# 17LiQi/MultimodalSignal

Hardware: AMD Instinct MI355X
Metric: train windows/sec (higher is better)
Workload: dtype f32; 1 GPU; CnnGruAttentionModel full train step (fwd+CE+bwd+Adam, dropout 0.5, BN batch stats), B=8192 windows/GPU x (6 ch, 3840 samples = 60 s @ 64 Hz), random-init weights; BASELINE.json configs[4] shape, the per-step work of configs[1]; batch_per_gpu=8192, channels=6, samples=3840, classes=2, parallelism=replica x1

## Files before the change

### multimodalsignal_amd/csrc/gru_bwd4.h

```cpp
#pragma once
template <int I> struct BwdB4 {
  static constexpr bool L1K = (I == 128);
  static constexpr int SD = 288;
  static constexpr int SX = L1K ? 224 : 96;
  static constexpr int DGP = 16 * SD, XHP = 16 * SX;
  static constexpr int BUFE = 3 * DGP + 3 * XHP;
  static constexpr int NPC = 6, NST = L1K ? 2 : 3;
  static constexpr int STG0 = 2 * BUFE * 2;
  static constexpr int SLOTB = 4 * NPC * 1024;
  static constexpr int SMEM = STG0 + NST * SLOTB;
};
struct BwdB6 {
  static constexpr int SD = 288, SX = 96, DGP = 16 * SD, XHP = 16 * SX;
  static constexpr int DGBUF = 3 * DGP, XHBUF = 3 * XHP;
  static constexpr int XH0 = 2 * DGBUF, NXH = 4;
  static constexpr int HNH0 = (XH0 + NXH * XHBUF) * 2;
  static constexpr int STG0 = HNH0 + 2 * 4096;
  static constexpr int NPC = 4, NST = 2, SLOTB = 4 * NPC * 1024;
  static constexpr int WHN0 = STG0 + NST * SLOTB;
  static constexpr int SMEM = WHN0 + 2 * 12288;
};
struct GruArgs;
struct FoldCtx;
int launch_gru_bwd_b4(int I, bool folds, const GruArgs& a, int n_tiles, int nwg, int ndir, const FoldCtx& fc, hipStream_t st, bool waves8 = false);
int launch_gru_bwd_seq4(int dh_mode, const GruArgs& a, int n_tiles, int ndir, const FoldCtx& fc, hipStream_t st);
int launch_gru_bwd_seq4_dw1(const GruArgs& a, const GruArgs& a1, int n_tiles, int nwg1, const FoldCtx& fc, hipStream_t st);
int gru_bwd_b4_lds_optin();
int launch_gru_bwd_b6(bool folds, const GruArgs& a, int n_tiles, int nwg, int ndir, const FoldCtx& fc, hipStream_t st);
int gru_bwd_b6_lds_optin();
```

### multimodalsignal_amd/csrc/gru_bwd6.hip

```cpp
#include "gru_args.h"
#include "gru_bwd4.h"
#include "gru_bwd_pipe.h"

template <bool FOLDS, int ROLE>
__device__ __forceinline__ void bwd6_run(const GruArgs& a, const GruDir& D, const float* __restrict__ ax_, const uint32_t dkey, const int n_tiles) {
  using G = BwdB6;
  constexpr int I = 32;
  constexpr bool CH = ROLE == 0, BA = ROLE == 1, BB = ROLE == 2;
  constexpr int SD = G::SD, SX = G::SX, DGP = G::DGP, XHP = G::XHP, DGBUF = G::DGBUF, XHBUF = G::XHBUF, XH0 = G::XH0;
  extern __shared__ __attribute__((aligned(16))) __bf16 ring[];
  constexpr int NT = BA ? 3 : (BB ? 6 : 0), NTA = NT > 0 ? NT : 1;
  constexpr int NST = G::NST, SLOTB = G::SLOTB, NPIECE = 4;
  const int tid = threadIdx.x, lane = tid & 63, w = (tid >> 6) & 3, li = lane & 15, lq = lane >> 4;
  const int u0 = w * 16 + lq * 4;

  bf16x8 AhB[CH ? 6 : 1][3], AiB[BA ? 6 : 1][3];
  if constexpr (CH || BA) {
#pragma unroll
    for (int kb = 0; kb < 6; ++kb)
#pragma unroll
      for (int j = 0; j < 8; ++j) {
        __bf16 p0, p1, p2;
        if constexpr (CH) {
          split3(D.Whh[(size_t)(kb * 32 + lq * 8 + j) * 64 + w * 16 + li], p0, p1, p2);
          AhB[kb][0][j] = p0; AhB[kb][1][j] = p1; AhB[kb][2][j] = p2;
        } else {
          split3(D.Wih[(size_t)(kb * 32 + lq * 8 + j) * I + w * 16 + li], p0, p1, p2);
          AiB[kb][0][j] = p0; AiB[kb][1][j] = p1; AiB[kb][2][j] = p2;
        }
      }
#pragma unroll
    for (int kb = 0; kb < 6; ++kb)
#pragma unroll
      for (int pp = 0; pp < 3; ++pp) { if constexpr (CH) PIN_ACC(AhB[kb][pp]); else PIN_ACC(AiB[kb][pp]); }
  }
  f32x4 b_hn[2] = {{0.f, 0.f, 0.f, 0.f}, {0.f, 0.f, 0.f, 0.f}};
  char* const whn = (char*)ring + G::WHN0 + (w & 1) * 12288 + lane * 16;
  if constexpr (BA) {
#pragma unroll
    for (int ub = 0; ub < 2; ++ub) {
#pragma unroll
      for (int kb = 0; kb < 2; ++kb) {
        const float* wr = D.Whh + (size_t)(128 + (w + 2 * ub) * 16 + li) * 64 + kb * 32 + lq * 8;
        bf16x8 P[3];
#pragma unroll
        for (int j = 0; j < 8; ++j) { __bf16 p0, p1, p2; split3(wr[j], p0, p1, p2); P[0][j] = p0; P[1][j] = p1; P[2][j] = p2; }
#pragma unroll
        for (int pp = 0; pp < 3; ++pp) *(bf16x8*)(whn + ((ub * 2 + kb) * 3 + pp) * 1024) = P[pp];
      }
#pragma unroll
      for (int e = 0; e < 4; ++e) b_hn[ub][e] = D.bhh[128 + (w + 2 * ub) * 16 + lq * 4 + e];
    }
  }
  int aoff[NTA], boff[NTA];
  aoff[0] = boff[0] = 0;
  if constexpr (BA) {
    aoff[0] = 192 + 32 * w; boff[0] = 0;
    aoff[1] = 128 + 32 * w; boff[1] = 32;
    aoff[2] = 128 + 32 * w; boff[2] = 64;
  } else if constexpr (BB) {
    const int gc = (w - 2) * 64;
#pragma unroll
    for (int t = 0; t < 6; ++t) { aoff[t] = gc + 32 * (t / 3); boff[t] = 32 * (t % 3); }
  }
  f32x16 accW[NTA];
#pragma unroll
  for (int t = 0; t < NT; ++t)
#pragma unroll
    for (int r = 0; r < 16; ++r) accW[t][r] = 0.f;
  float bacc[4][4];
#pragma unroll
  for (int g = 0; g < 4; ++g)
#pragma unroll
    for (int e = 0; e < 4; ++e) bacc[g][e] = 0.f;

  const int n_steps = D.n_steps, t_start = D.t_start, t_sign = D.t_sign;
  const int dthr = a.drop_thr;
  const float dscale = a.drop_scale;
  const int64_t h_bs = D.h_bs, h_ts = D.h_ts, dh_bs = D.dh_bs, dh_ts = D.dh_ts, x_bs = a.x_bs, x_ts = a.x_ts;
  const int64_t dx_bs = D.dx_bs, dx_ts = D.dx_ts;
  const int dh_col = D.dh_col;
  const int64_t hstep = (int64_t)t_sign * h_ts, ustep = (int64_t)t_sign * dh_ts;
  const int64_t dxstep = (int64_t)t_sign * dx_ts;

  const int sw_li = quad_swz(li);
  const int rd_row = li * SD + ((lq * 8) ^ sw_li);
  const int wr_dg = li * SD + (u0 ^ sw_li);
  const int rd_h = li * SX + ((I + lq * 8) ^ sw_li);
  int tr_dg[2], tr_xh[2];
  {
    const int g2 = lane >> 5, half = (lane >> 4) & 1;
#pragma unroll
    for (int h = 0; h < 2; ++h) {
      const int row = 8 * g2 + 4 * h + (li >> 2), sw = ((4 - (2 * g2 + h)) & 3) * 8;
      tr_dg[h] = row * SD + ((16 * half + 4 * (li & 3)) ^ sw);
      tr_xh[h] = row * SX + ((16 * half + 4 * (li & 3)) ^ sw);
    }
  }
  const int tb = tid & 127;
  const int sx_row = tb >> 3, sx_c4 = tb & 7;
  const int sx_off = sx_row * SX + ((4 * sx_c4) ^ quad_swz(sx_row));
  int sh_row[2], sh_c4[2], sh_off[2];
#pragma unroll
  for (int v = 0; v < 2; ++v) {
    const int idx = tb + 128 * v;
    sh_row[v] = idx >> 4; sh_c4[v] = idx & 15;
    sh_off[v] = sh_row[v] * SX + ((I + 4 * sh_c4[v]) ^ quad_swz(sh_row[v]));
  }
  char* const stg = (char*)ring + G::STG0 + lane * 16 + w * (NPIECE * 1024);
  const uint32_t stg_m0 = __builtin_amdgcn_readfirstlane((uint32_t)(uintptr_t)(ring) + G::STG0 + w * (NPIECE * 1024));
  char* const hnh = (char*)ring + G::HNH0 + lane * 16;
  auto xh_buf = [](int s) { return XH0 + (s & 3) * XHBUF; };

  for (int tile = blockIdx.x; tile < n_tiles; tile += gridDim.x) {
    const int tl = t_start + t_sign * (n_steps - 1);
    const int b = tile * 16 + li;
    const bool valid = b < a.B;
    const int bl = valid ? b : a.B - 1;
    const float vmask = valid ? 1.0f : 0.0f;
    const float sc_u = dscale * vmask;
    const int row0 = min(tile * 16, a.B - 1);
    auto uniform = [](const void* p) -> const char* {
      const uint64_t v = (uint64_t)(uintptr_t)p;
      const uint32_t lo = __builtin_amdgcn_readfirstlane((uint32_t)v), hi = __builtin_amdgcn_readfirstlane((uint32_t)(v >> 32));
      return (const char*)(uintptr_t)(((uint64_t)hi << 32) | lo);
    };
    [[maybe_unused]] const char* sp_b = uniform(D.stash + ((size_t)((size_t)tile * n_steps + (n_steps - 1)) * 4 + w) * 4 * 64);
    [[maybe_unused]] const uint32_t sp_off = (uint32_t)lane * 16;
    [[maybe_unused]] const char* hq_b = uniform(D.h + D.h_col + (int64_t)row0 * h_bs + (int64_t)(n_steps > 1 ? tl - t_sign : tl) * h_ts);
    [[maybe_unused]] const uint32_t hq_off = (uint32_t)(((int64_t)(bl - row0) * h_bs + u0) * 4);
    [[maybe_unused]] const char* uq_b = uniform(D.dh + D.dh_col + (int64_t)row0 * dh_bs + (int64_t)tl * dh_ts);
    [[maybe_unused]] const uint32_t uq_off = (uint32_t)(((int64_t)(bl - row0) * dh_bs + u0) * 4);
    [[maybe_unused]] uint32_t ue = (uint32_t)((int64_t)bl * dh_bs + (int64_t)tl * dh_ts + dh_col + u0);
    [[maybe_unused]] float4 hcur = make_float4(0.f, 0.f, 0.f, 0.f);
    if constexpr (CH) hcur = *(const float4*)(D.h + D.h_col + u0 + (int64_t)bl * h_bs + (int64_t)tl * h_ts);
    [[maybe_unused]] float* dxq = D.dx + lq * 4 + (int64_t)b * dx_bs + (int64_t)tl * dx_ts;
    auto dma = [&](const uint32_t voff, const char* sbase, const uint32_t lds_dst) {
      asm volatile("s_mov_b32 m0, %2\n\ts_nop 0\n\tglobal_load_lds_dwordx4 %0, %1" :: "v"(voff), "s"(sbase), "s"(lds_dst) : "memory");
    };
    auto load_piece = [&](int i, int s, int slot) {
      const uint32_t dst = stg_m0 + slot * SLOTB;
      if (i == 0) dma(sp_off, sp_b, dst);
      if (i == 1) { dma(sp_off, sp_b + 64 * 16, dst + 1024); if (s > 0) sp_b -= 4 * 4 * 64 * 16; }
      if (i == 2) { dma(hq_off, hq_b, dst + 2048); if (s > 1) hq_b -= hstep * 4; }
      if (i == 3) { dma(uq_off, uq_b, dst + 3072); if (s > 0) uq_b -= ustep * 4; }
    };
    auto issue_loads = [&](int s, int slot) {
#pragma unroll
      for (int i = 0; i < NPIECE; ++i) load_piece(i, s, slot);
    };
    struct Staged { float4 r4, z4, hn4, hp4, up4; uint32_t ue; float hkeep; };
    int cons_left = n_steps;
    int cons_step = 0;
    auto read_staged = [&](Staged& L, int slot) {
      const char* q = stg + slot * SLOTB;
      L.r4 = *(const float4*)q; L.z4 = *(const float4*)(q + 1024); L.hp4 = *(const float4*)(q + 2048); L.up4 = *(const float4*)(q + 3072);
      L.hn4 = *(const float4*)(hnh + 4096 * (cons_step & 1) + 1024 * w);
      L.ue = ue; ue -= (uint32_t)ustep;
      L.hkeep = cons_left == 1 ? 0.0f : 1.0f;
      --cons_left; ++cons_step;
    };
    auto clamp0 = [](int s) { return s > 0 ? s : 0; };

    struct XH { f32x4 x, h[2]; };
    auto gload = [](const float* p) -> f32x4 { f32x4 v; asm volatile("global_load_dwordx4 %0, %1, off" : "=v"(v) : "v"(p) : "memory"); return v; };
    const int sxb = min(tile * 16 + sx_row, a.B - 1);
    const float* sx_p = ax_ + (int64_t)sxb * x_bs + 4 * sx_c4;
    const float* sh_p[2];
#pragma unroll
    for (int v = 0; v < 2; ++v) sh_p[v] = D.h + D.h_col + (int64_t)min(tile * 16 + sh_row[v], a.B - 1) * h_bs + 4 * sh_c4[v];
    auto load_xh = [&](XH& R, int s, auto asyncc) {
      constexpr bool ASYNC = decltype(asyncc)::value;
      const int sc = s < n_steps ? s : n_steps - 1, t = tl - t_sign * sc, tp = sc < n_steps - 1 ? t - t_sign : t;
      if constexpr (ASYNC) {
        R.x = gload(sx_p + (int64_t)t * x_ts);
#pragma unroll
        for (int v = 0; v < 2; ++v) R.h[v] = gload(sh_p[v] + (int64_t)tp * h_ts);
      } else {
        R.x = *(const f32x4*)(sx_p + (int64_t)t * x_ts);
#pragma unroll
        for (int v = 0; v < 2; ++v) R.h[v] = *(const f32x4*)(sh_p[v] + (int64_t)tp * h_ts);
      }
    };
    auto xh_wait = [](XH& R) {
      asm volatile("s_waitcnt vmcnt(3)" : "+v"(R.x), "+v"(R.h[0]), "+v"(R.h[1]) :: "memory");
    };
    auto zero_last = [&](XH& R, int s) {
      if (s >= n_steps - 1) { R.h[0] = (f32x4){0.f, 0.f, 0.f, 0.f}; R.h[1] = R.h[0]; }
    };
    float hk = 1.0f;
    auto stage_now = [&](const XH& R, int s) {
      const int xb = xh_buf(s);
      bf16x4 p[3];
      split3_quad(R.x, p);
#pragma unroll
      for (int pp = 0; pp < 3; ++pp) *(bf16x4*)&ring[xb + pp * XHP + sx_off] = p[pp];
#pragma unroll
      for (int v = 0; v < 2; ++v) {
        split3_quad(R.h[v], p);
#pragma unroll
        for (int pp = 0; pp < 3; ++pp) *(bf16x4*)&ring[xb + pp * XHP + sh_off[v]] = p[pp];
      }
    };
    auto hn_block = [&](int s) {
      const __bf16* pb = ring + xh_buf(s) + rd_h;
      bf16x8 ho[2][3], Al[2][2][3];
#pragma unroll
      for (int kb = 0; kb < 2; ++kb)
#pragma unroll
        for (int pp = 0; pp < 3; ++pp) {
          ho[kb][pp] = *(const bf16x8*)&pb[pp * XHP + kb * 32];
#pragma unroll
          for (int ub = 0; ub < 2; ++ub) Al[ub][kb][pp] = *(const bf16x8*)(whn + ((ub * 2 + kb) * 3 + pp) * 1024);
        }
#pragma unroll
      for (int ub = 0; ub < 2; ++ub) {
        f32x4 acc = b_hn[ub];
#pragma unroll
        for (int kb = 0; kb < 2; ++kb) acc = mfma_bf16x3<CT_FWD_REC>(Al[ub][kb], ho[kb], acc);
        *(float4*)(hnh + 4096 * (s & 1) + 1024 * (w + 2 * ub)) = make_float4(acc[0], acc[1], acc[2], acc[3]);
      }
    };

    float cN[4], cZ[4], cR[4], rv[4], zv[4], upm[4] = {0.f, 0.f, 0.f, 0.f}, hpv[4], t0[4], t1[4], t2[4], t3[4], dhv[4];
    float dhz[4] = {0.f, 0.f, 0.f, 0.f};
    float dgv[4][4];
    SplitPair spg[2], spx[3][2];
    uint32_t wd_u = 0;
    f32x4 dh_next = {0.f, 0.f, 0.f, 0.f};
    constexpr int NC_ = 60, NU_ = 14, NQ1 = NC_ + NU_;
    auto q1 = [&](auto kc, Staged& L) {
      constexpr int K = decltype(kc)::value;
      if constexpr (K < NC_) {
        constexpr int S = K / 4, e = K % 4;
        const float r_ = f4e<e>(L.r4), z_ = f4e<e>(L.z4), hh_ = f4e<e>(L.hn4), hc_ = f4e<e>(hcur);
        if constexpr (S == 0) { hpv[e] = f4e<e>(L.hp4) * L.hkeep; PINV(hpv[e]); }
        if constexpr (S == 1) { t0[e] = 1.0f - z_; PINV(t0[e]); }
        if constexpr (S == 2) { t1[e] = __builtin_fmaf(-z_, hpv[e], hc_); PINV(t1[e]); }
        if constexpr (S == 3) { t2[e] = __builtin_fmaxf(t0[e], 1e-30f); PINV(t2[e]); }
        if constexpr (S == 4) { t2[e] = __builtin_amdgcn_rcpf(t2[e]); PINV(t2[e]); }
        if constexpr (S == 5) { t3[e] = 1.0f - r_; PINV(t3[e]); }
        if constexpr (S == 6) { t3[e] = r_ * t3[e]; PINV(t3[e]); }
        if constexpr (S == 7) { cR[e] = hh_ * t3[e]; PINV(cR[e]); }
        if constexpr (S == 8) { t3[e] = z_ * t0[e]; PINV(t3[e]); }
        if constexpr (S == 9) { t1[e] = t1[e] * t2[e]; PINV(t1[e]); }
        if constexpr (S == 10) { t1[e] = __builtin_amdgcn_fmed3f(t1[e], -1.0f, 1.0f); PINV(t1[e]); }
        if constexpr (S == 11) { t2[e] = __builtin_fmaf(-t1[e], t1[e], 1.0f); PINV(t2[e]); }
        if constexpr (S == 12) { cN[e] = t0[e] * t2[e]; PINV(cN[e]); }
        if constexpr (S == 13) { t2[e] = hpv[e] - t1[e]; PINV(t2[e]); }
        if constexpr (S == 14) { cZ[e] = t2[e] * t3[e]; rv[e] = r_; zv[e] = z_; PINV(cZ[e]); }
      } else {
        constexpr int S = K - NC_;
        if constexpr (S == 0) wd_u = (L.ue >> 2) ^ dkey;
        if constexpr (S == 1) wd_u ^= wd_u >> 16;
        if constexpr (S == 2) wd_u *= 0x85EBCA6Bu;
        if constexpr (S == 3) wd_u ^= wd_u >> 13;
        if constexpr (S == 4) wd_u *= 0xC2B2AE35u;
        if constexpr (S == 5) wd_u ^= wd_u >> 16;
        if constexpr (S < 6) PINV(wd_u);
        if constexpr (S >= 6 && S < 10) { upm[S - 6] = drop_mul(wd_u, S - 6, dthr, sc_u); PINV(upm[S - 6]); }
        if constexpr (S >= 10) { upm[S - 10] = upm[S - 10] * f4e<S - 10>(L.up4); PINV(upm[S - 10]); }
      }
    };
    constexpr int NDM = 24, NBA = 16, NG1 = 2 * SPLIT_STAGES + 3, NQ2 = NDM + NBA + 4 * NG1;
    auto q2 = [&](auto kc, const int nb) {
      constexpr int K = decltype(kc)::value;
      if constexpr (K < NDM) {
        constexpr int S = K / 4, e = K % 4;
        if constexpr (S == 0) { dhv[e] = dh_next[e] + upm[e]; PINV(dhv[e]); }
        if constexpr (S == 1) { dhz[e] = dhv[e] * zv[e]; PINV(dhz[e]); }
        if constexpr (S == 2) { dgv[3][e] = dhv[e] * cN[e]; PINV(dgv[3][e]); }
        if constexpr (S == 3) { dgv[1][e] = dhv[e] * cZ[e]; PINV(dgv[1][e]); }
        if constexpr (S == 4) { dgv[0][e] = dgv[3][e] * cR[e]; PINV(dgv[0][e]); }
        if constexpr (S == 5) { dgv[2][e] = dgv[3][e] * rv[e]; PINV(dgv[2][e]); }
      } else if constexpr (K < NDM + NBA) {
        constexpr int g = (K - NDM) / 4, e = (K - NDM) % 4;
        bacc[g][e] += dgv[g][e];
        PINV(bacc[g][e]);
      } else {
        constexpr int gi = (K - NDM - NBA) / NG1, S = (K - NDM - NBA) % NG1;
        constexpr int g = gi == 0 ? 1 : (gi == 1 ? 3 : (gi == 2 ? 0 : 2));
        if constexpr (S < 2 * SPLIT_STAGES) {
          constexpr int st = S / 2, p = S % 2;
          if constexpr (st == 0) { spg[p].a = dgv[g][2 * p]; spg[p].b = dgv[g][2 * p + 1]; }
          split_stage<st>(spg[p]);
        } else {
          constexpr int pp = S - 2 * SPLIT_STAGES;
          *(uint2*)&ring[nb + wr_dg + pp * DGP + g * 64] = make_uint2(spg[0].P[pp], spg[1].P[pp]);
        }
      }
    };
    constexpr int NX1 = 2 * SPLIT_STAGES + 3, NQX = 3 * NX1;
    auto qx = [&](auto kc, const XH& R, const int xb) {
      constexpr int K = decltype(kc)::value, v = K / NX1, S0 = K % NX1;
      if constexpr (S0 < 2 * SPLIT_STAGES) {
        constexpr int st = S0 / 2, p = S0 % 2;
        if constexpr (st == 0) {
          const f32x4& q = v == 0 ? R.x : R.h[v == 0 ? 0 : v - 1];
          if constexpr (v == 0) { spx[v][p].a = q[2 * p]; spx[v][p].b = q[2 * p + 1]; }
          else { spx[v][p].a = q[2 * p] * hk; spx[v][p].b = q[2 * p + 1] * hk; }
        }
        split_stage<st>(spx[v][p]);
      } else {
        constexpr int pp = S0 - 2 * SPLIT_STAGES;
        const int off = v == 0 ? sx_off : sh_off[v == 0 ? 0 : v - 1];
        *(uint2*)&ring[xb + off + pp * XHP] = make_uint2(spx[v][0].P[pp], spx[v][1].P[pp]);
      }
    };

    int cur = 0, nxt = DGBUF;
    STAMP_DECL;
    Staged L;
    XH RA, RB;
    int slot_c = 0, steps_issued = 0;
    if constexpr (CH) {
#pragma unroll
      for (int q = 0; q < NST; ++q) { issue_loads(clamp0(n_steps - 1 - q), q); ++steps_issued; }
    }
    if constexpr (BB) {
#pragma unroll
      for (int s = 0; s < 3; ++s) { load_xh(RA, s, std::false_type{}); zero_last(RA, s); stage_now(RA, s); }
      FENCE();
      load_xh(RA, 3, std::true_type{});
    }
    lds_barrier();
    if constexpr (BA) {
      hn_block(0);
      if (n_steps > 1) hn_block(1);
    }
    lds_barrier();
    if constexpr (CH) {
      WAIT_VM((NST - 1) * NPIECE);
      read_staged(L, 0);
      sfor<NQ1>([&](auto k) { q1(k, L); });
      hcur = L.hp4;
      sfor<NQ2>([&](auto k) { q2(k, cur); });
      dh_next = (f32x4){0.f, 0.f, 0.f, 0.f};
      FENCE();
      issue_loads(clamp0(n_steps - 1 - steps_issued), 0); ++steps_issued;
      slot_c = 1 % NST;
    }
    lds_barrier();

    auto step = [&](auto fullc, const int j, XH& Rc, XH& Rl) {
      constexpr bool FULL = decltype(fullc)::value;
      STAMP(0);
      if constexpr (CH) {
        if constexpr (FULL) {
          const int s_ld = clamp0(n_steps - 1 - steps_issued);
          const __bf16* pb = ring + cur + rd_row;
          bf16x8 q[6][3];
          auto rd_rec = [&](auto kbc) {
            constexpr int kb = decltype(kbc)::value;
#pragma unroll
            for (int pp = 0; pp < 3; ++pp) q[kb][pp] = *(const bf16x8*)&pb[pp * DGP + kb * 32];
          };
          WAIT_VM((NST - 1) * NPIECE);
          read_staged(L, slot_c);
          sfor<3>(rd_rec);
          FENCE();
          constexpr int PRE = 2, RF0 = 8;
          sfor<PRE>([&](auto k) { q1(k, L); });
          FENCE();
          STAMP(1);
          f32x4 ah0 = {0.f, 0.f, 0.f, 0.f}, ah1 = {0.f, 0.f, 0.f, 0.f};
          sfor<36>([&](auto sc) {
            constexpr int s = decltype(sc)::value, kb = s / 6, t = s % 6;
            if constexpr (kb & 1) { ah1 = mf16<t, CT_BWD_REC>(AhB[kb], q[kb], ah1); PINA(ah1); } else { ah0 = mf16<t, CT_BWD_REC>(AhB[kb], q[kb], ah0); PINA(ah0); }
            FENCE();
            if constexpr (t == 0 && kb + 3 < 6) rd_rec(ic<kb + 3>{});
            if constexpr (s == RF0 - 1) { PINV(L.r4.x); PINV(L.z4.x); PINV(L.hp4.x); PINV(L.up4.x); PINV(L.hn4.x); }
            if constexpr (s >= RF0 && s < RF0 + NPIECE) load_piece(s - RF0, s_ld, slot_c);
            if constexpr (PRE + 2 * s < NQ1) q1(ic<PRE + 2 * s>{}, L);
            if constexpr (PRE + 2 * s + 1 < NQ1) q1(ic<PRE + 2 * s + 1>{}, L);
            FENCE();
          });
          static_assert(NQ1 <= PRE + 72, "the coefficients must be complete before the dependent part starts");
#pragma unroll
          for (int e = 0; e < 4; ++e) dh_next[e] = dhz[e] + ah0[e] + ah1[e];
          hcur = L.hp4;
          ++steps_issued; slot_c = slot_c + 1 == NST ? 0 : slot_c + 1;
          FENCE();
          STAMP(2);
          sfor<NQ2>([&](auto k) { q2(k, nxt); });
          STAMP(3);
        }
        lds_barrier();
        STAMP(5);
        { const int o = cur; cur = nxt; nxt = o; }
        return;
      }
      if constexpr (BB && FULL) { load_xh(Rl, j + 4, std::true_type{}); hk = j + 3 >= n_steps - 1 ? 0.0f : 1.0f; FENCE(); }
      const __bf16* pb = ring + cur + rd_row;
      const int xcur = xh_buf(j);
      constexpr int NBR = BA ? 2 : 3, NFR = 6 * NBR + 12;
      bf16x8 Af[2][3], Bf[NBR][3];
      auto frag_read = [&](auto nc) {
        constexpr int n = decltype(nc)::value;
        if constexpr (n < 6 * NBR) {
          constexpr int blk = n / 6, pp = (n % 6) / 2, h = n % 2;
          put_half<h>(Bf[blk][pp], lds_tr_read4(ring + xcur + tr_xh[h] + 32 * blk + pp * XHP));
        } else if constexpr (n < NFR) {
          constexpr int m = n - 6 * NBR, blk = m / 6, pp = (m % 6) / 2, h = m % 2;
          put_half<h>(Af[blk][pp], lds_tr_read4(ring + cur + tr_dg[h] + aoff[BB ? 3 * blk : blk] + pp * DGP));
        }
      };
      [[maybe_unused]] const int xnew = xh_buf(j + 3);
      [[maybe_unused]] f32x4 ax;
      if constexpr (BB) {
        sfor<NFR>(frag_read);
        FENCE();
        if constexpr (FULL) { xh_wait(Rc); FENCE(); }
      }
      if constexpr (BA) {
        ax = (f32x4){0.f, 0.f, 0.f, 0.f};
        bf16x8 qd[3][3];
        auto rd_dx = [&](auto kbc) {
          constexpr int kb = decltype(kbc)::value, col0 = kb < 4 ? kb * 32 : 192 + (kb - 4) * 32;
#pragma unroll
          for (int pp = 0; pp < 3; ++pp) qd[kb % 3][pp] = *(const bf16x8*)&pb[pp * DGP + col0];
        };
        bf16x8 hoq[2][3], Alq[2][3];
        f32x4 hacc = b_hn[0];
        auto rd_al = [&](auto gc) {
          constexpr int g = decltype(gc)::value, ub = g / 2, kb = g % 2;
#pragma unroll
          for (int pp = 0; pp < 3; ++pp) Alq[g & 1][pp] = *(const bf16x8*)(whn + ((ub * 2 + kb) * 3 + pp) * 1024);
        };
        if constexpr (FULL) {
          const __bf16* ph = ring + xh_buf(j + 2) + rd_h;
#pragma unroll
          for (int kb = 0; kb < 2; ++kb)
#pragma unroll
            for (int pp = 0; pp < 3; ++pp) hoq[kb][pp] = *(const bf16x8*)&ph[pp * XHP + kb * 32];
          rd_al(ic<0>{});
        }
        rd_dx(ic<0>{});
        rd_dx(ic<1>{});
        FENCE();
        sfor<36>([&](auto sc) {
          constexpr int s = decltype(sc)::value, kb = s / 6, t = s % 6;
          if constexpr (FULL && s < 24) {
            constexpr int g = s / 6, ub = g / 2, hkb = g % 2;
            hacc = mf16<t, CT_FWD_REC>(Alq[g & 1], hoq[hkb], hacc);
            PINA(hacc);
            FENCE();
            if constexpr (t == 0 && g + 1 < 4) rd_al(ic<g + 1>{});
            if constexpr (s % 12 == 11) {
              *(float4*)(hnh + 4096 * ((j + 2) & 1) + 1024 * (w + 2 * ub)) = make_float4(hacc[0], hacc[1], hacc[2], hacc[3]);
              hacc = b_hn[1];
            }
          }
          ax = mf16<t, CT_DX>(AiB[kb], qd[kb % 3], ax);
          PINA(ax);
          FENCE();
          if constexpr (t == 0 && kb + 2 < 6) rd_dx(ic<kb + 2>{});
          if constexpr (FULL) {
            if constexpr (s >= 24) { frag_read(ic<2 * (s - 24)>{}); frag_read(ic<2 * (s - 24) + 1>{}); }
          } else {
            if constexpr (s >= 2 && s < 2 + NFR) frag_read(ic<s - 2>{});
          }
          FENCE();
        });
        static_assert(NFR == 24, "bulk A: 24 fragment reads in the last 12 dX slots");
      }
      STAMP(3);
      sfor<6 * NT>([&](auto sc) {
        constexpr int s = decltype(sc)::value, tI = s / 6, t = s % 6;
        constexpr int ai = BA ? (tI == 0 ? 0 : 1) : tI / 3;
        constexpr int bi = BA ? (tI == 1 ? 1 : 0) : tI % 3;
        accW[tI] = mf32<t, CT_DW>(Af[ai], Bf[bi], accW[tI]);
        PINA(accW[tI]);
        FENCE();
        if constexpr (BA && tI == 1) put_half<t % 2>(Bf[0][t / 2], lds_tr_read4(ring + xcur + tr_xh[t % 2] + 64 + (t / 2) * XHP));
        if constexpr (BA && s == 1) {
          if (valid) *(float4*)(dxq + w * 16) = make_float4(ax[0], ax[1], ax[2], ax[3]);
          dxq -= dxstep;
        }
        if constexpr (BB && FULL) {
          sfor<6>([&](auto oc) {
            constexpr int K = 6 * s + decltype(oc)::value;
            if constexpr (K < NQX) qx(ic<K>{}, Rc, xnew);
          });
        }
        FENCE();
      });
      static_assert(NQX <= 36 * 6, "not enough MFMA gaps for the staging of a step");
      STAMP(4);
      lds_barrier();
      STAMP(5);
      { const int o = cur; cur = nxt; nxt = o; }
    };
    const int n_full = n_steps - 1;
    for (int j = 0; j < n_full; j += 2) {
      step(std::true_type{}, j, RA, RB);
      if (j + 1 < n_full) step(std::true_type{}, j + 1, RB, RA);
    }
    if constexpr (BB) WAIT_VM(0);
    step(std::false_type{}, n_full, RA, RB);
    if constexpr (CH) WAIT_VM(0);
#ifdef MSIG_STAMPS
    constexpr int rec = ROLE;
    if (a.dbg && lane == 0 && w == (BB ? 2 : 0) && tile == (int)blockIdx.x)
      for (int i = 0; i < 8; ++i) a.dbg[(((size_t)rec * gridDim.y + blockIdx.y) * gridDim.x + blockIdx.x) * 8 + i] = ph_[i];
#endif
  }

  float* Pp = D.part + (size_t)blockIdx.x * (192 * I + 192 * 64 + 256);
#pragma unroll
  for (int t = 0; t < NT; ++t) {
    const int ao = aoff[t], bo = boff[t];
    const int row0 = ao < 192 ? ao : ao - 64;
    const bool ih = bo < I;
    float* base = ih ? Pp + (size_t)row0 * I + bo : Pp + 192 * I + (size_t)row0 * 64 + (bo - I);
    const int ld = ih ? I : 64;
#pragma unroll
    for (int r = 0; r < 16; ++r) base[(size_t)(8 * (r >> 2) + 4 * (lane >> 5) + (r & 3)) * ld + (lane & 31)] = accW[t][r];
  }
  float* scratch = (float*)ring;
  constexpr int RSB = 272;
  if constexpr (CH) {
#pragma unroll
    for (int g = 0; g < 4; ++g) *(float4*)&scratch[li * RSB + g * 64 + u0] = make_float4(bacc[g][0], bacc[g][1], bacc[g][2], bacc[g][3]);
  }
  lds_barrier();
  if constexpr (CH) {
    float bsum = 0.f;
#pragma unroll
    for (int r = 0; r < 16; ++r) bsum += scratch[r * RSB + tid];
    Pp[192 * I + 192 * 64 + (tid < 128 ? tid : (tid < 192 ? tid + 64 : tid - 64))] = bsum;
  }
}

template <bool FOLDS>
__global__ __launch_bounds__(512, 1) void gru_bwd_b6(const GruArgs a, int n_tiles, const FoldCtx fc) {
  FOLD_GRU_ARGS_IF(FOLDS);
  (void)axkey_;
  if (threadIdx.x < 256) bwd6_run<FOLDS, 0>(a, D, ax_, akey_, n_tiles);
  else if (threadIdx.x < 384) bwd6_run<FOLDS, 1>(a, D, ax_, akey_, n_tiles);
  else bwd6_run<FOLDS, 2>(a, D, ax_, akey_, n_tiles);
}

int gru_bwd_b6_lds_optin() {
  const hipFuncAttribute A = hipFuncAttributeMaxDynamicSharedMemorySize;
  hipError_t e;
  if ((e = hipFuncSetAttribute((const void*)gru_bwd_b6<false>, A, BwdB6::SMEM)) != hipSuccess) return (int)e;
  if ((e = hipFuncSetAttribute((const void*)gru_bwd_b6<true>, A, BwdB6::SMEM)) != hipSuccess) return (int)e;
  return 0;
}

int launch_gru_bwd_b6(bool folds, const GruArgs& a, int n_tiles, int nwg, int ndir, const FoldCtx& fc, hipStream_t st) {
  const dim3 grid(nwg, ndir, folds ? fc.n : 1);
  if (folds) gru_bwd_b6<true><<<grid, 512, BwdB6::SMEM, st>>>(a, n_tiles, fc);
  else gru_bwd_b6<false><<<grid, 512, BwdB6::SMEM, st>>>(a, n_tiles, fc);
  MSIG_LAUNCH_CHECK();
#ifdef MSIG_STAMPS
  if (a.dbg) {
    (void)hipStreamSynchronize(st);
    static unsigned long long h[3 * 2 * 256 * 8];
    const int per = ndir * nwg;
    (void)hipMemcpy(h, a.dbg, sizeof(unsigned long long) * 8 * 3 * per, hipMemcpyDeviceToHost);
    const char* names[3] = {"chain wave 0", "bulk wave 4 (hn, dX, 3 dW tiles)", "bulk wave 6 (6 dW tiles, x / h staging)"};
    for (int role = 0; role < 3; ++role) {
      double acc[8] = {0};
      for (int i = 0; i < per; ++i) for (int j = 0; j < 8; ++j) acc[j] += (double)h[((size_t)role * per + i) * 8 + j] / per;
      const double steps = a.dir[0].n_steps;
      if (role == 0)
        fprintf(stderr, "[stamps b6 %s, cycles per step (first tile)] loop top %.0f | wait + staged reads %.0f | recurrence %.0f | dependent gate math + stores %.0f | barrier %.0f\n",
                names[role], acc[0] / steps, acc[1] / steps, acc[2] / steps, acc[3] / steps, acc[5] / steps);
      else
        fprintf(stderr, "[stamps b6 %s, cycles per step (first tile)] loop top %.0f | hn + fragment reads + dX %.0f | dW %.0f | barrier %.0f\n",
                names[role], acc[0] / steps, acc[3] / steps, acc[4] / steps, acc[5] / steps);
    }
  }
#endif
  return 0;
}
```

### multimodalsignal_amd/csrc/gru_bwd_pipe.h

```cpp
#pragma once
#include "gru_args.h"

typedef float f32x16 __attribute__((ext_vector_type(16)));
#define LDS_AS __attribute__((address_space(3)))
#define FENCE() do { asm volatile("" ::: "memory"); __builtin_amdgcn_sched_barrier(0); } while (0)
#define PIN_ACC(v) asm volatile("" : "+a"(v))
#define PINA(v) asm volatile("" : "+a"(v))
#define PINV(v) asm volatile("" : "+v"(v))
#define WAIT_VM(n) asm volatile("s_waitcnt vmcnt(%0)" :: "n"(n) : "memory")

template <int N> using ic = std::integral_constant<int, N>;
template <typename F, int... Is> __device__ __forceinline__ void sfor_impl(F&& f, std::integer_sequence<int, Is...>) { (f(ic<Is>{}), ...); }
template <int N, typename F> __device__ __forceinline__ void sfor(F&& f) { sfor_impl(f, std::make_integer_sequence<int, N>{}); }

__device__ __forceinline__ bf16x4 lds_tr_read4(const __bf16* p) {
  typedef __attribute__((__vector_size__(4 * sizeof(__bf16)))) __bf16 v4;
  const v4 r = __builtin_amdgcn_ds_read_tr16_b64_v4bf16((LDS_AS v4*)p);
  return __builtin_bit_cast(bf16x4, r);
}
template <int T, int KIND> __device__ __forceinline__ f32x4 mf16(const bf16x8 (&a)[3], const bf16x8 (&b)[3], f32x4 acc) {
  constexpr int ai[6] = {2, 0, 1, 1, 0, 0}, bi[6] = {0, 2, 1, 0, 1, 0};
  if constexpr (T == 2 && msig_drop_ct<KIND>()) return acc;
  return __builtin_amdgcn_mfma_f32_16x16x32_bf16(a[ai[T]], b[bi[T]], acc, 0, 0, 0);
}
template <int T, int KIND> __device__ __forceinline__ f32x16 mf32(const bf16x8 (&a)[3], const bf16x8 (&b)[3], f32x16 acc) {
  constexpr int ai[6] = {2, 0, 1, 1, 0, 0}, bi[6] = {0, 2, 1, 0, 1, 0};
  if constexpr (T == 2 && msig_drop_ct<KIND>()) return acc;
  return __builtin_amdgcn_mfma_f32_32x32x16_bf16(a[ai[T]], b[bi[T]], acc, 0, 0, 0);
}
__device__ __forceinline__ uint32_t top_pair_u(uint32_t a, uint32_t b) { return __builtin_amdgcn_perm(b, a, 0x07060302u); }

struct SplitPair { float a, b; uint32_t ta, tb, P[3]; };
template <int S> __device__ __forceinline__ void split_stage(SplitPair& s) {
  if constexpr (S == 0) { s.P[0] = top_pair_u(__float_as_uint(s.a), __float_as_uint(s.b)); PINV(s.P[0]); }
  if constexpr (S == 1 || S == 6) { s.ta = __float_as_uint(s.a) & 0xFFFF0000u; PINV(s.ta); }
  if constexpr (S == 2 || S == 7) { s.tb = __float_as_uint(s.b) & 0xFFFF0000u; PINV(s.tb); }
  if constexpr (S == 3 || S == 8) { s.a = s.a - __uint_as_float(s.ta); PINV(s.a); }
  if constexpr (S == 4 || S == 9) { s.b = s.b - __uint_as_float(s.tb); PINV(s.b); }
  if constexpr (S == 5) { s.P[1] = top_pair_u(__float_as_uint(s.a), __float_as_uint(s.b)); PINV(s.P[1]); }
  if constexpr (S == 10) { s.P[2] = top_pair_u(__float_as_uint(s.a), __float_as_uint(s.b)); PINV(s.P[2]); }
}
constexpr int SPLIT_STAGES = 11;


template <int E> __device__ __forceinline__ float f4e(const float4& v) {
  if constexpr (E == 0) return v.x; else if constexpr (E == 1) return v.y; else if constexpr (E == 2) return v.z; else return v.w;
}
template <int E> __device__ __forceinline__ void f4mul(float4& v, float m) {
  if constexpr (E == 0) v.x *= m; else if constexpr (E == 1) v.y *= m; else if constexpr (E == 2) v.z *= m; else v.w *= m;
}
template <int H> __device__ __forceinline__ void put_half(bf16x8& f, const bf16x4 v) {
  f[4 * H + 0] = v[0]; f[4 * H + 1] = v[1]; f[4 * H + 2] = v[2]; f[4 * H + 3] = v[3];
}
```

Baseline: 1.049 million windows/s.

## Switch GRU backward hn recompute from bf16x3 to scaled f16x2 MFMA split

Replaces the three-way bf16 split of the recurrent hn weights and hidden state with a two-way scaled fp16 split. The product now takes three MFMAs per block instead of six, and the MFMAs are rescaled after accumulation. A separate double-buffered f16 hidden-state LDS region and staging path are added, and the hn MFMAs are interleaved into the dX slots at a configurable stride. This cuts MFMA and LDS read work in the BA role. It risks numeric differences from the per-row scaling and adds LDS footprint and extra split/store work in the BB role.

```diff
diff --git a/multimodalsignal_amd/csrc/gru_bwd4.h b/multimodalsignal_amd/csrc/gru_bwd4.h
--- a/multimodalsignal_amd/csrc/gru_bwd4.h
+++ b/multimodalsignal_amd/csrc/gru_bwd4.h
@@ -18,7 +18,11 @@
   static constexpr int STG0 = HNH0 + 2 * 4096;
   static constexpr int NPC = 4, NST = 2, SLOTB = 4 * NPC * 1024;
   static constexpr int WHN0 = STG0 + NST * SLOTB;
-  static constexpr int SMEM = WHN0 + 2 * 12288;
+  static constexpr int WHNB = 2 * 2 * 2 * 1024;
+  static constexpr int SH = 96, H16P = 16 * SH, H16BUF = 2 * H16P;
+  static constexpr int H160 = WHN0 + 2 * WHNB;
+  static constexpr int SMEM = H160 + 2 * H16BUF * 2;
+  static_assert(SMEM <= 160 * 1024, "gru_bwd_b6: more LDS than a gfx950 workgroup can have");
 };
 struct GruArgs;
 struct FoldCtx;
diff --git a/multimodalsignal_amd/csrc/gru_bwd6.hip b/multimodalsignal_amd/csrc/gru_bwd6.hip
--- a/multimodalsignal_amd/csrc/gru_bwd6.hip
+++ b/multimodalsignal_amd/csrc/gru_bwd6.hip
@@ -35,18 +35,27 @@
       for (int pp = 0; pp < 3; ++pp) { if constexpr (CH) PIN_ACC(AhB[kb][pp]); else PIN_ACC(AiB[kb][pp]); }
   }
   f32x4 b_hn[2] = {{0.f, 0.f, 0.f, 0.f}, {0.f, 0.f, 0.f, 0.f}};
-  char* const whn = (char*)ring + G::WHN0 + (w & 1) * 12288 + lane * 16;
+  float post[2] = {0.f, 0.f};
+  char* const whn = (char*)ring + G::WHN0 + (w & 1) * G::WHNB + lane * 16;
   if constexpr (BA) {
 #pragma unroll
     for (int ub = 0; ub < 2; ++ub) {
+      float wv[2][8], m = 0.f;
 #pragma unroll
       for (int kb = 0; kb < 2; ++kb) {
         const float* wr = D.Whh + (size_t)(128 + (w + 2 * ub) * 16 + li) * 64 + kb * 32 + lq * 8;
-        bf16x8 P[3];
-#pragma unroll
-        for (int j = 0; j < 8; ++j) { __bf16 p0, p1, p2; split3(wr[j], p0, p1, p2); P[0][j] = p0; P[1][j] = p1; P[2][j] = p2; }
-#pragma unroll
-        for (int pp = 0; pp < 3; ++pp) *(bf16x8*)(whn + ((ub * 2 + kb) * 3 + pp) * 1024) = P[pp];
+#pragma unroll
+        for (int j = 0; j < 8; ++j) { wv[kb][j] = wr[j]; m = fmaxf(m, fabsf(wv[kb][j])); }
+      }
+      const float sw = f16x2_weight_scale(m);
+      post[ub] = 1.0f / (sw * F16X2_H_SCALE);
+#pragma unroll
+      for (int kb = 0; kb < 2; ++kb) {
+        f16x8 P[2];
+#pragma unroll
+        for (int j = 0; j < 8; ++j) { _Float16 p0, p1; split2(wv[kb][j], sw, p0, p1); P[0][j] = p0; P[1][j] = p1; }
+#pragma unroll
+        for (int pp = 0; pp < 2; ++pp) *(f16x8*)(whn + ((ub * 2 + kb) * 2 + pp) * 1024) = P[pp];
       }
 #pragma unroll
       for (int e = 0; e < 4; ++e) b_hn[ub][e] = D.bhh[128 + (w + 2 * ub) * 16 + lq * 4 + e];
@@ -86,7 +95,8 @@
   const int sw_li = quad_swz(li);
   const int rd_row = li * SD + ((lq * 8) ^ sw_li);
   const int wr_dg = li * SD + (u0 ^ sw_li);
-  const int rd_h = li * SX + ((I + lq * 8) ^ sw_li);
+  _Float16* const h16 = (_Float16*)((char*)ring + G::H160);
+  const int rd_h16 = li * G::SH + ((lq * 8) ^ sw_li);
   int tr_dg[2], tr_xh[2];
   {
     const int g2 = lane >> 5, half = (lane >> 4) & 1;
@@ -100,12 +110,13 @@
   const int tb = tid & 127;
   const int sx_row = tb >> 3, sx_c4 = tb & 7;
   const int sx_off = sx_row * SX + ((4 * sx_c4) ^ quad_swz(sx_row));
-  int sh_row[2], sh_c4[2], sh_off[2];
+  int sh_row[2], sh_c4[2], sh_off[2], sh16_off[2];
 #pragma unroll
   for (int v = 0; v < 2; ++v) {
     const int idx = tb + 128 * v;
     sh_row[v] = idx >> 4; sh_c4[v] = idx & 15;
     sh_off[v] = sh_row[v] * SX + ((I + 4 * sh_c4[v]) ^ quad_swz(sh_row[v]));
+    sh16_off[v] = sh_row[v] * G::SH + ((4 * sh_c4[v]) ^ quad_swz(sh_row[v]));
   }
   char* const stg = (char*)ring + G::STG0 + lane * 16 + w * (NPIECE * 1024);
   const uint32_t stg_m0 = __builtin_amdgcn_readfirstlane((uint32_t)(uintptr_t)(ring) + G::STG0 + w * (NPIECE * 1024));
@@ -202,22 +213,33 @@
         for (int pp = 0; pp < 3; ++pp) *(bf16x4*)&ring[xb + pp * XHP + sh_off[v]] = p[pp];
       }
     };
+    auto split_h16 = [&](const XH& R, f16x4 (&p)[2][2]) {
+#pragma unroll
+      for (int v = 0; v < 2; ++v) split2_quad(R.h[v], F16X2_H_SCALE, p[v][0], p[v][1]);
+    };
+    auto store_h16 = [&](const f16x4 (&p)[2][2], int s) {
+#pragma unroll
+      for (int v = 0; v < 2; ++v)
+#pragma unroll
+        for (int pp = 0; pp < 2; ++pp) *(f16x4*)&h16[(s & 1) * G::H16BUF + pp * G::H16P + sh16_off[v]] = p[v][pp];
+    };
     auto hn_block = [&](int s) {
-      const __bf16* pb = ring + xh_buf(s) + rd_h;
-      bf16x8 ho[2][3], Al[2][2][3];
+      const _Float16* ph = h16 + (s & 1) * G::H16BUF + rd_h16;
+      f16x8 ho[2][2], Al[2][2][2];
 #pragma unroll
       for (int kb = 0; kb < 2; ++kb)
 #pragma unroll
-        for (int pp = 0; pp < 3; ++pp) {
-          ho[kb][pp] = *(const bf16x8*)&pb[pp * XHP + kb * 32];
-#pragma unroll
-          for (int ub = 0; ub < 2; ++ub) Al[ub][kb][pp] = *(const bf16x8*)(whn + ((ub * 2 + kb) * 3 + pp) * 1024);
+        for (int pp = 0; pp < 2; ++pp) {
+          ho[kb][pp] = *(const f16x8*)&ph[pp * G::H16P + kb * 32];
+#pragma unroll
+          for (int ub = 0; ub < 2; ++ub) Al[ub][kb][pp] = *(const f16x8*)(whn + ((ub * 2 + kb) * 2 + pp) * 1024);
         }
 #pragma unroll
       for (int ub = 0; ub < 2; ++ub) {
-        f32x4 acc = b_hn[ub];
-#pragma unroll
-        for (int kb = 0; kb < 2; ++kb) acc = mfma_bf16x3<CT_FWD_REC>(Al[ub][kb], ho[kb], acc);
+        f32x4 acc = {0.f, 0.f, 0.f, 0.f};
+#pragma unroll
+        for (int kb = 0; kb < 2; ++kb) acc = mfma_f16x2<CT_FWD_REC>(Al[ub][kb], ho[kb], acc);
+        acc = b_hn[ub] + acc * post[ub];
         *(float4*)(hnh + 4096 * (s & 1) + 1024 * (w + 2 * ub)) = make_float4(acc[0], acc[1], acc[2], acc[3]);
       }
     };
@@ -290,10 +312,20 @@
         }
       }
     };
-    constexpr int NX1 = 2 * SPLIT_STAGES + 3, NQX = 3 * NX1;
-    auto qx = [&](auto kc, const XH& R, const int xb) {
-      constexpr int K = decltype(kc)::value, v = K / NX1, S0 = K % NX1;
-      if constexpr (S0 < 2 * SPLIT_STAGES) {
+    constexpr int NX1 = 2 * SPLIT_STAGES + 3, NXB = 3 * NX1, NH1 = 6, NQX = NXB + 2 * NH1;
+    struct Split2Q { f32x4 t; f16x4 hi, lo; } s2[2];
+    auto qx = [&](auto kc, const XH& R, const int xb, const int hb) {
+      constexpr int K = decltype(kc)::value;
+      if constexpr (K >= NXB) {
+        constexpr int v = (K - NXB) / NH1, S = (K - NXB) % NH1;
+        if constexpr (S == 0) { s2[v].t = R.h[v] * (hk * F16X2_H_SCALE); PINV(s2[v].t); }
+        if constexpr (S == 1) { s2[v].hi = __builtin_convertvector(s2[v].t, f16x4); PINV(s2[v].hi); }
+        if constexpr (S == 2) { s2[v].t = s2[v].t - __builtin_convertvector(s2[v].hi, f32x4); PINV(s2[v].t); }
+        if constexpr (S == 3) { s2[v].lo = __builtin_convertvector(s2[v].t, f16x4); PINV(s2[v].lo); }
+        if constexpr (S == 4) *(f16x4*)&h16[hb + sh16_off[v]] = s2[v].hi;
+        if constexpr (S == 5) *(f16x4*)&h16[hb + G::H16P + sh16_off[v]] = s2[v].lo;
+      } else if constexpr (K % NX1 < 2 * SPLIT_STAGES) {
+        constexpr int v = K / NX1, S0 = K % NX1;
         constexpr int st = S0 / 2, p = S0 % 2;
         if constexpr (st == 0) {
           const f32x4& q = v == 0 ? R.x : R.h[v == 0 ? 0 : v - 1];
@@ -302,6 +334,7 @@
         }
         split_stage<st>(spx[v][p]);
       } else {
+        constexpr int v = K / NX1, S0 = K % NX1;
         constexpr int pp = S0 - 2 * SPLIT_STAGES;
         const int off = v == 0 ? sx_off : sh_off[v == 0 ? 0 : v - 1];
         *(uint2*)&ring[xb + off + pp * XHP] = make_uint2(spx[v][0].P[pp], spx[v][1].P[pp]);
@@ -317,9 +350,14 @@
 #pragma unroll
       for (int q = 0; q < NST; ++q) { issue_loads(clamp0(n_steps - 1 - q), q); ++steps_issued; }
     }
+    [[maybe_unused]] f16x4 hp2[2][2];
     if constexpr (BB) {
 #pragma unroll
-      for (int s = 0; s < 3; ++s) { load_xh(RA, s, std::false_type{}); zero_last(RA, s); stage_now(RA, s); }
+      for (int s = 0; s < 3; ++s) {
+        load_xh(RA, s, std::false_type{}); zero_last(RA, s); stage_now(RA, s);
+        split_h16(RA, hp2);
+        if (s < 2) store_h16(hp2, s);
+      }
       FENCE();
       load_xh(RA, 3, std::true_type{});
     }
@@ -329,6 +367,7 @@
       if (n_steps > 1) hn_block(1);
     }
     lds_barrier();
+    if constexpr (BB) store_h16(hp2, 2);
     if constexpr (CH) {
       WAIT_VM((NST - 1) * NPIECE);
       read_staged(L, 0);
@@ -405,7 +444,7 @@
           put_half<h>(Af[blk][pp], lds_tr_read4(ring + cur + tr_dg[h] + aoff[BB ? 3 * blk : blk] + pp * DGP));
         }
       };
-      [[maybe_unused]] const int xnew = xh_buf(j + 3);
+      [[maybe_unused]] const int xnew = xh_buf(j + 3), h16new = ((j + 3) & 1) * G::H16BUF;
       [[maybe_unused]] f32x4 ax;
       if constexpr (BB) {
         sfor<NFR>(frag_read);
@@ -420,49 +459,56 @@
 #pragma unroll
           for (int pp = 0; pp < 3; ++pp) qd[kb % 3][pp] = *(const bf16x8*)&pb[pp * DGP + col0];
         };
-        bf16x8 hoq[2][3], Alq[2][3];
-        f32x4 hacc = b_hn[0];
-        auto rd_al = [&](auto gc) {
-          constexpr int g = decltype(gc)::value, ub = g / 2, kb = g % 2;
-#pragma unroll
-          for (int pp = 0; pp < 3; ++pp) Alq[g & 1][pp] = *(const bf16x8*)(whn + ((ub * 2 + kb) * 3 + pp) * 1024);
+#ifndef MSIG_B6_HN_STRIDE
+#define MSIG_B6_HN_STRIDE 2
+#endif
+#ifndef MSIG_B6_FR0
+#define MSIG_B6_FR0 12
+#endif
+        constexpr int HN_STRIDE = MSIG_B6_HN_STRIDE, FR0 = MSIG_B6_FR0, FRN = NFR / (36 - FR0);
+        static_assert(12 * HN_STRIDE <= 36 && FRN * (36 - FR0) == NFR, "bulk A: 12 hn MFMAs and 24 fragment reads in 36 dX slots");
+        f16x8 hoq[2][2], Alq[4][2];
+        f32x4 hacc = {0.f, 0.f, 0.f, 0.f};
+        [[maybe_unused]] const _Float16* ph = h16 + ((j + 2) & 1) * G::H16BUF + rd_h16;
+        auto rd_hn = [&](auto gc) {
+          constexpr int g = decltype(gc)::value;
+#pragma unroll
+          for (int pp = 0; pp < 2; ++pp) {
+            if constexpr (g < 2) hoq[g][pp] = *(const f16x8*)&ph[pp * G::H16P + g * 32];
+            Alq[g][pp] = *(const f16x8*)(whn + (g * 2 + pp) * 1024);
+          }
         };
-        if constexpr (FULL) {
-          const __bf16* ph = ring + xh_buf(j + 2) + rd_h;
-#pragma unroll
-          for (int kb = 0; kb < 2; ++kb)
-#pragma unroll
-            for (int pp = 0; pp < 3; ++pp) hoq[kb][pp] = *(const bf16x8*)&ph[pp * XHP + kb * 32];
-          rd_al(ic<0>{});
-        }
+        if constexpr (FULL) rd_hn(ic<0>{});
         rd_dx(ic<0>{});
+        if constexpr (FULL) rd_hn(ic<1>{});
         rd_dx(ic<1>{});
+        if constexpr (FULL) { rd_hn(ic<2>{}); rd_hn(ic<3>{}); }
         FENCE();
         sfor<36>([&](auto sc) {
           constexpr int s = decltype(sc)::value, kb = s / 6, t = s % 6;
-          if constexpr (FULL && s < 24) {
-            constexpr int g = s / 6, ub = g / 2, hkb = g % 2;
-            hacc = mf16<t, CT_FWD_REC>(Alq[g & 1], hoq[hkb], hacc);
+          constexpr bool HN = FULL && s % HN_STRIDE == 0 && s / HN_STRIDE < 12;
+          constexpr int hs = s / HN_STRIDE, g = HN ? hs / 3 : 0;
+          if constexpr (HN) {
+            hacc = mfh16<hs % 3, CT_FWD_REC>(Alq[g], hoq[g % 2], hacc);
             PINA(hacc);
             FENCE();
-            if constexpr (t == 0 && g + 1 < 4) rd_al(ic<g + 1>{});
-            if constexpr (s % 12 == 11) {
-              *(float4*)(hnh + 4096 * ((j + 2) & 1) + 1024 * (w + 2 * ub)) = make_float4(hacc[0], hacc[1], hacc[2], hacc[3]);
-              hacc = b_hn[1];
-            }
           }
           ax = mf16<t, CT_DX>(AiB[kb], qd[kb % 3], ax);
           PINA(ax);
           FENCE();
+          if constexpr (HN && hs % 6 == 5) {
+            const f32x4 hv = b_hn[g / 2] + hacc * post[g / 2];
+            *(float4*)(hnh + 4096 * ((j + 2) & 1) + 1024 * (w + 2 * (g / 2))) = make_float4(hv[0], hv[1], hv[2], hv[3]);
+            hacc = (f32x4){0.f, 0.f, 0.f, 0.f};
+          }
           if constexpr (t == 0 && kb + 2 < 6) rd_dx(ic<kb + 2>{});
           if constexpr (FULL) {
-            if constexpr (s >= 24) { frag_read(ic<2 * (s - 24)>{}); frag_read(ic<2 * (s - 24) + 1>{}); }
+            if constexpr (s >= FR0) sfor<FRN>([&](auto ic_) { frag_read(ic<FRN * (s - FR0) + decltype(ic_)::value>{}); });
           } else {
             if constexpr (s >= 2 && s < 2 + NFR) frag_read(ic<s - 2>{});
           }
           FENCE();
         });
-        static_assert(NFR == 24, "bulk A: 24 fragment reads in the last 12 dX slots");
       }
       STAMP(3);
       sfor<6 * NT>([&](auto sc) {
@@ -480,7 +526,7 @@
         if constexpr (BB && FULL) {
           sfor<6>([&](auto oc) {
             constexpr int K = 6 * s + decltype(oc)::value;
-            if constexpr (K < NQX) qx(ic<K>{}, Rc, xnew);
+            if constexpr (K < NQX) qx(ic<K>{}, Rc, xnew, h16new);
           });
         }
         FENCE();
diff --git a/multimodalsignal_amd/csrc/gru_bwd_pipe.h b/multimodalsignal_amd/csrc/gru_bwd_pipe.h
--- a/multimodalsignal_amd/csrc/gru_bwd_pipe.h
+++ b/multimodalsignal_amd/csrc/gru_bwd_pipe.h
@@ -28,6 +28,11 @@
   if constexpr (T == 2 && msig_drop_ct<KIND>()) return acc;
   return __builtin_amdgcn_mfma_f32_32x32x16_bf16(a[ai[T]], b[bi[T]], acc, 0, 0, 0);
 }
+template <int T, int KIND> __device__ __forceinline__ f32x4 mfh16(const f16x8 (&a)[2], const f16x8 (&b)[2], f32x4 acc) {
+  constexpr int ai[3] = {1, 0, 0}, bi[3] = {0, 1, 0};
+  if constexpr (T == 0 && msig_drop_ct<KIND>()) return acc;
+  return __builtin_amdgcn_mfma_f32_16x16x32_f16(a[ai[T]], b[bi[T]], acc, 0, 0, 0);
+}
 __device__ __forceinline__ uint32_t top_pair_u(uint32_t a, uint32_t b) { return __builtin_amdgcn_perm(b, a, 0x07060302u); }
 
 struct SplitPair { float a, b; uint32_t ta, tb, P[3]; };
```

After: 1.058 million windows/s (median of 4 runs). Within noise of the previous version (+0.8%).
